# kylittle/Crucible

Hardware: AMD Instinct MI355X
Metric: Msamples/sec (whole node) + achieved HBM GB/s, book1 1920×1080 @ 1/2/4/8 GPU (higher is better)
Workload: dtype f64

## Files before the change

crucible_amd/csrc/pathtrace.hpp:

```cpp
#pragma once
#include <hip/hip_runtime.h>
#include <stddef.h>
#include <stdint.h>
#include <type_traits>

#define CR_HD __host__ __device__ __forceinline__
#define CR_D __device__ __forceinline__
#include "fastdiv.hpp"
#include "residency.hpp"

namespace cr {

template <typename real> struct RealTraits;
template <> struct RealTraits<float> {
    static constexpr float eps = 1.1920928955078125e-07f;
    static constexpr float tiny = 0.0f;
    static constexpr float pi = 3.14159265358979323846f;
};
template <> struct RealTraits<double> {
    static constexpr double eps = 2.220446049250313e-16;
    static constexpr double tiny = 1e-160;
    static constexpr double pi = 3.14159265358979323846;
};

// ... 283 lines not shown
    f.from = from;
    V3<real> w = unit(sub(from, at));
    V3<real> u = unit(cross(c.vup, w));
    V3<real> v = cross(w, u);
    V3<real> vu = scale(c.viewport_width, u);
    V3<real> vv = scale(c.viewport_height, neg(v));
    f.pdu = divs(vu, (real)c.W);
    f.pdv = divs(vv, (real)c.H);
    V3<real> ul = sub(from, scale(c.focus_dist, w));
    ul = sub(ul, divs(vu, real(2)));
    ul = sub(ul, divs(vv, real(2)));
    f.p00 = add(ul, scale(real(0.5), add(f.pdu, f.pdv)));
    f.ddu = scale(c.defocus_radius, u);
    f.ddv = scale(c.defocus_radius, v);
    return f;
}

#if defined(__HIPCC__)

#ifdef CR_DIAG
enum { DG_BOX_WAVE = 0, DG_BOX_LANE, DG_PRIM_WAVE, DG_PRIM_LANE, DG_ROUND_WAVE, DG_ROUND_LANE, DG_LEAFPH_WAVE, DG_LEAFPH_LANE,
       DG_SHADE_WAVE, DG_SHADE_LANE, DG_LAMB_LANE, DG_METAL_LANE, DG_DIEL_LANE, DG_SKY_LANE, DG_RUV_WAVE, DG_RUV_LANE,
       DG_REGEN_WAVE, DG_REGEN_LANE, DG_OUTER_WAVE, DG_UNWIND_WAVE, DG_UNWIND_LANE, DG_HITSH_WAVE, DG_HITSH_LANE, DG_BAND_WAVE, DG_BAND_LANE,
       DG_ROOT2_WAVE, DG_ROOT2_LANE, DG_QUOT_WAVE, DG_QUOT_LANE, DG_QUOTDIV_WAVE, DG_QUOTDIV_LANE, DG_N };
struct Diag { uint32_t v[DG_N]; };
#define CR_DIAG_LEADER() ((threadIdx.x & 63u) == (uint32_t)(__ffsll((unsigned long long)__ballot(1)) - 1))
#define CR_DIAG_HIT(dg, wave_i, lane_i) do { if (dg) { (dg)->v[lane_i]++; if (CR_DIAG_LEADER()) (dg)->v[wave_i]++; } } while (0)
#define CR_DIAG_LANE(dg, lane_i) do { if (dg) (dg)->v[lane_i]++; } while (0)
#else
struct Diag {};
#define CR_DIAG_HIT(dg, wave_i, lane_i) ((void)0)
#define CR_DIAG_LANE(dg, lane_i) ((void)0)
#endif

template <typename real> struct Hit {
    real t;
    int32_t prim;
};

template <typename real>
CR_D bool box_hit(const real* b, V3<real> o, V3<real> inv, real tmin, real tmax) {
    real t0 = (b[0] - o.x) * inv.x, t1 = (b[1] - o.x) * inv.x;
    real nmin, nmax;
    if (t0 < t1) { nmin = t0 > tmin ? t0 : tmin; nmax = t1 < tmax ? t1 : tmax; }
    else { nmin = t1 > tmin ? t1 : tmin; nmax = t0 < tmax ? t0 : tmax; }
    tmin = nmin; tmax = nmax;
    t0 = (b[2] - o.y) * inv.y; t1 = (b[3] - o.y) * inv.y;
// ... 226 lines not shown
template <typename real> CR_HD real soft_acos(real x) {
    using K = TrigK<real>;
    const real ax = r_abs(x);
    if (ax < real(0.5)) { const real z = x * x; return K::pio2_hi - (x - (K::pio2_lo - x * (z * K::S(z)))); }
    if (!(ax <= real(1))) return (x - x) / (x - x);
    if (x < real(0)) {
        const real t = (real(1) + x) * real(0.5);
        const real s = r_sqrt(t);
        const real w = (t * K::S(t)) * s - K::pio2_lo;
        return K::pi_hi - real(2) * (s + w);
    }
    const real t = (real(1) - x) * real(0.5);
    const real s = r_sqrt(t);
    return real(2) * (s + s * (t * K::S(t)));
}
CR_D float r_atan2(float y, float x) { return soft_atan2(y, x); }
CR_D float r_asin(float x) { return soft_asin(x); }
CR_D float r_acos(float x) { return soft_acos(x); }
#define CR_D_CALL static __device__ __attribute__((noinline))
CR_D_CALL double r_atan2(double y, double x) { return soft_atan2(y, x); }
CR_D_CALL double r_asin(double x) { return soft_asin(x); }
CR_D_CALL double r_acos(double x) { return soft_acos(x); }

CR_D float screen_coord(uint64_t u) {
    return (float)((int32_t)(uint32_t)(u >> 40) - (int32_t)(1 << 23)) * 0x1.0p-23f;
}
template <typename real> CR_D V3<real> random_unit_vector_dev(uint64_t& s) {
    if constexpr (!std::is_same<real, double>::value) return random_unit_vector<real>(s);
    else {
        uint64_t ux, uy, uz;
        for (;;) {
            ux = rng_next(s); uy = rng_next(s); uz = rng_next(s);
            const float fx = screen_coord(ux), fy = screen_coord(uy), fz = screen_coord(uz);
            const float lf = __builtin_fmaf(fz, fz, __builtin_fmaf(fy, fy, fx * fx));
            if (lf > 1.0f + 1e-5f) continue;
            if (lf > 1e-5f && lf < 1.0f - 1e-5f) break;
            const double x = -1.0 + 2.0 * u01(ux, 0.0), y = -1.0 + 2.0 * u01(uy, 0.0), z = -1.0 + 2.0 * u01(uz, 0.0);
            const double lensq = x * x + y * y + z * z;
            if (RealTraits<double>::tiny < lensq && lensq <= 1.0) break;
        }
        const V3<double> p = mk<double>(-1.0 + 2.0 * u01(ux, 0.0), -1.0 + 2.0 * u01(uy, 0.0), -1.0 + 2.0 * u01(uz, 0.0));
        return divs(p, r_sqrt(len2(p)));
    }
}
template <typename real> CR_D void random_in_unit_disk_dev(uint64_t& s, real& px, real& py) {
    if constexpr (!std::is_same<real, double>::value) {
        for (;;) {
            px = rng_range<real>(s, real(-1), real(1));
            py = rng_range<real>(s, real(-1), real(1));
            if (px * px + py * py + real(0) * real(0) < real(1)) break;
        }
    } else {
        uint64_t ux, uy;
        for (;;) {
            ux = rng_next(s); uy = rng_next(s);
            const float fx = screen_coord(ux), fy = screen_coord(uy);
            const float lf = __builtin_fmaf(fy, fy, fx * fx);
            if (lf > 1.0f + 1e-5f) continue;
            if (lf < 1.0f - 1e-5f) break;
            const double x = -1.0 + 2.0 * u01(ux, 0.0), y = -1.0 + 2.0 * u01(uy, 0.0);
            if (x * x + y * y + 0.0 * 0.0 < 1.0) break;
        }
        px = -1.0 + 2.0 * u01(ux, 0.0); py = -1.0 + 2.0 * u01(uy, 0.0);
    }
}

template <typename real, bool ANIM, bool CAMK = false>
CR_D void camera_ray(const KernelArgs<real>& A, uint32_t pix_i, uint32_t pix_j, int32_t sample, uint64_t& rng, V3<real>& ro, V3<real>& rd,
                     real& rtime, real current_time) {
    const CamConst<real>& cam = A.cam;
    uint32_t pixel = pix_j * (uint32_t)cam.W + pix_i;
    rng = rng_key(A.seed_mixed, pixel, (uint32_t)sample);
    real ts = current_time + rng_range<real>(rng, real(0), A.shutter_length);
    real ox = rng_uniform<real>(rng) - real(0.5);
    real oy = rng_uniform<real>(rng) - real(0.5);
    CamFrame<real> f;
    if ((ANIM || CAMK) && cam.animated) {
        real fx = cam.from.x, fy = cam.from.y, fz = cam.from.z, fw = real(1);
        real ax = cam.at.x, ay = cam.at.y, az = cam.at.z, aw = real(1);
        timeline_eval(A.cam_keys + cam.from_key_first, cam.from_key_count, ts, fx, fy, fz, fw);
        timeline_eval(A.cam_keys + cam.at_key_first, cam.at_key_count, ts, ax, ay, az, aw);
        f = camera_frame(cam, mk<real>(fw * fx, fw * fy, fw * fz), mk<real>(aw * ax, aw * ay, aw * az));
    } else {
        f.from = cam.from; f.p00 = cam.p00; f.pdu = cam.pdu; f.pdv = cam.pdv; f.ddu = cam.ddu; f.ddv = cam.ddv;
    }
    V3<real> ps = add(add(f.p00, scale((real)pix_i + ox, f.pdu)), scale((real)pix_j + oy, f.pdv));
    V3<real> orig = f.from;
    if (cam.defocus_on) {
        real px, py;
        random_in_unit_disk_dev<real>(rng, px, py);
        orig = add(add(f.from, scale(px, f.ddu)), scale(py, f.ddv));
    }
    ro = orig; rd = sub(ps, orig); rtime = ts;
}
template <typename real, bool ANIM, bool CAMK = false>
CR_D void camera_ray(const KernelArgs<real>& A, uint32_t pix_i, uint32_t pix_j, int32_t sample, uint64_t& rng, V3<real>& ro, V3<real>& rd,
                     real& rtime) {
    camera_ray<real, ANIM, CAMK>(A, pix_i, pix_j, sample, rng, ro, rd, rtime, A.current_time);
}

template <typename T> CR_D T load_rec(const T* p, bool in_lds) {
    static_assert(sizeof(T) % 4 == 0, "records are whole words");
    T out;
    uint32_t* o = reinterpret_cast<uint32_t*>(&out);
    if (in_lds) {
        const __attribute__((address_space(3))) uint32_t* s = (const __attribute__((address_space(3))) uint32_t*)(const void*)p;
        for (size_t k = 0; k < sizeof(T) / 4; k++) o[k] = s[k];
    } else {
        const __attribute__((address_space(1))) uint32_t* s = (const __attribute__((address_space(1))) uint32_t*)(const void*)p;
        for (size_t k = 0; k < sizeof(T) / 4; k++) o[k] = s[k];
    }
    return out;
}

#define CR_CHECKER_LEAF(tex_at, ti, tx, p)                                                                                          \
    for (int guard = 0; guard < 32 && tx.kind == 1; guard++) {                                                                   \
        int32_t s = (int32_t)((uint32_t)as_i32(r_floor(tx.inv_scale * p.x)) + (uint32_t)as_i32(r_floor(tx.inv_scale * p.y)) +   \
                              (uint32_t)as_i32(r_floor(tx.inv_scale * p.z)));                                                      \
        ti = (s % 2 == 0) ? tx.even : tx.odd;                                                                                    \
        tx = tex_at(ti);                                                                                                         \
    }

template <typename real, bool ANIM, bool SIDE_SPLIT = false, bool RELAX = false>
CR_D bool shade(const KernelArgs<real>& A, const Prim<real>* prims, const Mat<real>* mats, const Tex<real>* texs, V3<real>& ro, V3<real>& rd,
                real rtime, uint64_t& rng, int32_t& depth_left, int32_t& stack_n, real best_t, int32_t best, uint32_t stack_stride,
                uint32_t stack_slot, uint32_t& c_tex, V3<real>& col, Diag* dg = nullptr, V3<real>* thr = nullptr) {
    CR_DIAG_HIT(dg, DG_SHADE_WAVE, DG_SHADE_LANE);
    if (best >= 0) {
        CR_DIAG_HIT(dg, DG_HITSH_WAVE, DG_HITSH_LANE);
        const Prim<real>& p = prims[best];
        V3<real> loc = add(ro, scale(best_t, rd));
        V3<real> n;
        real tu = 0, tv = 0;
        auto mat_at = [&](int32_t i) { return SIDE_SPLIT ? load_rec(mats + i, A.lds_side != 0) : mats[i]; };
        auto tex_at = [&](int32_t i) { return SIDE_SPLIT ? load_rec(texs + i, A.lds_side != 0) : texs[i]; };
        const Mat<real> m = mat_at(p.mat());
        bool need_uv = false;
        int32_t leaf_tex = -1;
        if (m.kind == 0 && m.tex >= 0) {
            int ti = m.tex;
            Tex<real> tx = tex_at(ti);
            CR_CHECKER_LEAF(tex_at, ti, tx, loc)
            need_uv = tx.kind == 2;
            leaf_tex = ti;
        }
        if (p.kind() == 0) {
            real g0 = p.g[0], g1 = p.g[1], g2 = p.g[2], g3 = p.g[3];
            if (ANIM && p.key_count) {
                timeline_eval(A.keys + p.key_first, p.key_count, rtime, g0, g1, g2, g3);
                n = divs(sub(loc, mk<real>(g0, g1, g2)), g3);
            } else n = scale(p.g[4], sub(loc, mk<real>(g0, g1, g2)));
            if (need_uv) {
                real theta = r_acos(-n.y);
                real phi = r_atan2(-n.z, n.x) + RealTraits<real>::pi;
                tu = phi / (real(2) * RealTraits<real>::pi);
                tv = theta / RealTraits<real>::pi;
            }
        } else {
            V3<real> a = mk<real>(p.g[0], p.g[1], p.g[2]), b = mk<real>(p.g[3], p.g[4], p.g[5]), c = mk<real>(p.g[6], p.g[7], p.g[8]);
            if (ANIM && p.key_count) {
                a = timeline_vertex(A.keys + p.key_first, p.key_count, rtime, a);
                b = timeline_vertex(A.keys + p.key_first, p.key_count, rtime, b);
                c = timeline_vertex(A.keys + p.key_first, p.key_count, rtime, c);
            }
            n = unit(cross(sub(b, a), sub(c, a)));
            tu = 0; tv = 0;
        }
        bool front = dot(rd, n) < real(0);
        if (!front) n = neg(n);

        V3<real> att = mk<real>(0, 0, 0), ndir = rd;
        bool some;
        V3<real> ruv = mk<real>(0, 0, 0);
#ifdef CR_DIAG
        if (m.kind != 2) {
            for (;;) {
                CR_DIAG_HIT(dg, DG_RUV_WAVE, DG_RUV_LANE);
                real x = rng_range<real>(rng, real(-1), real(1)), y = rng_range<real>(rng, real(-1), real(1)), z = rng_range<real>(rng, real(-1), real(1));
                V3<real> pp = mk<real>(x, y, z);
                real lensq = len2(pp);
                if (RealTraits<real>::tiny < lensq && lensq <= real(1)) { ruv = divs(pp, r_sqrt(lensq)); break; }
            }
        }
        CR_DIAG_LANE(dg, m.kind == 0 ? DG_LAMB_LANE : (m.kind == 1 ? DG_METAL_LANE : DG_DIEL_LANE));
#else
        if (m.kind != 2) ruv = random_unit_vector_dev<real>(rng);
#endif
        if (m.kind == 0) {
            V3<real> dir = add(n, ruv);
            real tol = real(1e-8);
            if (r_abs(dir.x) < tol && r_abs(dir.y) < tol && r_abs(dir.z) < tol) dir = n;
            V3<real> tc;
            if (m.tex < 0) tc = mk<real>(m.albedo[0], m.albedo[1], m.albedo[2]);
            else {
                const Tex<real> lt = tex_at(leaf_tex);
                if (need_uv) tc = image_lookup(A.images, A.texels, lt.image, tu, tv, c_tex);
                else tc = mk<real>(lt.color[0], lt.color[1], lt.color[2]);
            }
            att = c_scale(m.aux, (m.param < real(0)) ? c_neg(tc) : tc);
            ndir = dir;
            if (__ballot(!(m.param >= real(1))) == 0ull) { rng_step(rng); some = true; }
            else some = rng_uniform<real>(rng) <= m.param;
        } else if (m.kind == 1) {
            V3<real> refl = reflect(rd, n);
            refl = add(unit(refl), scale(m.param, ruv));
            att = mk<real>(m.albedo[0], m.albedo[1], m.albedo[2]);
            ndir = refl;
            some = dot(refl, n) > real(0);
        } else {
            att = mk<real>(1, 1, 1);
// ... 164 lines not shown
}

template <typename real> struct WalkState {
    V3<real> inv;
    real dd;
    real rda;
    real best_t;
    int32_t best;
    int32_t idx;
    bool exact_box;
    int32_t oct;
    int32_t pending;
};

template <bool SHARED = false, typename real> CR_D void walk_begin(WalkState<real>& w, V3<real> rd) {
    w.inv = mk<real>(real(1) / rd.x, real(1) / rd.y, real(1) / rd.z);
    w.exact_box = (r_abs(w.inv.x) == r_inf(real(0))) || (r_abs(w.inv.y) == r_inf(real(0))) || (r_abs(w.inv.z) == r_inf(real(0)));
    w.dd = len2(rd);
    w.rda = SHARED ? shared_rcp(w.dd) : quot_divide<real>();
    w.idx = 0; w.best_t = r_inf(real(0)); w.best = -1; w.pending = -1;
    w.oct = (rd.x < real(0) ? 1 : 0) | (rd.y < real(0) ? 2 : 0) | (rd.z < real(0) ? 4 : 0);
}

CR_D void screen_extents(float ofx, float ofy, float ofz, float ifx, float ify, float ifz, float& mo, float& pmax, float& pmin) {
    mo = r_max(r_max(__builtin_fabsf(ofx), __builtin_fabsf(ofy)), __builtin_fabsf(ofz));
    pmax = r_max(r_max(__builtin_fabsf(ifx), __builtin_fabsf(ify)), __builtin_fabsf(ifz));
    pmin = r_min(r_min(__builtin_fabsf(ifx), __builtin_fabsf(ify)), __builtin_fabsf(ifz));
}
CR_D bool screen_in_range(bool exact_box, float mo, float pmax, float pmin) {
    return !exact_box && pmin >= 0x1.0p-100f && pmax <= 0x1.0p100f && mo <= 0x1.0p100f;
}
CR_D float screen_q(float of, float inv_f) { return __builtin_fabsf(of * inv_f); }
CR_D float screen_th0(float qx, float qy, float qz, float pmax) {
    return __builtin_fmaf(0x1.0p-20f, r_max(r_max(qx, qy), qz), __builtin_fmaf(pmax * 0x1.0p-100f, 0x1.0p-47f, 1e-35f));
}
CR_D float screen_box_d(const float* b, Pair<float> fox, Pair<float> foy, Pair<float> foz, Pair<float> fix, Pair<float> fiy, Pair<float> fiz,
                        float tminf, float tmaxf, float th0, float& th) {
    const Pair<float> tx = __builtin_elementwise_fma(Pair<float>{b[0], b[1]}, fix, -(fox * fix));
    const Pair<float> ty = __builtin_elementwise_fma(Pair<float>{b[2], b[3]}, fiy, -(foy * fiy));
    const Pair<float> tz = __builtin_elementwise_fma(Pair<float>{b[4], b[5]}, fiz, -(foz * fiz));
    const float nx = r_min(tx.x, tx.y), ny = r_min(ty.x, ty.y), nz = r_min(tz.x, tz.y);
    const float fx = r_max(tx.x, tx.y), fy = r_max(ty.x, ty.y), fz = r_max(tz.x, tz.y);
    const float lo = r_max(r_max(nx, ny), r_max(nz, tminf));
    float hi, m;
    asm("v_min_f32_e32 %0, %2, %3\n\tv_min3_f32 %0, %4, %5, %0\n\tv_max_f32_e64 %1, |%6|, |%0|"
        : "=&v"(hi), "=v"(m) : "v"(fz), "v"(tmaxf), "v"(fx), "v"(fy), "v"(lo));
    th = __builtin_fmaf(0x1.0p-20f, m, th0);
    return hi - lo;
}
CR_D bool screen_box_miss_exact(const float* b, Pair<float> fox, Pair<float> foy, Pair<float> foz, Pair<float> fix, Pair<float> fiy,
                                Pair<float> fiz, float tminf, float tmaxf) {
    const Pair<float> tx = (Pair<float>{b[0], b[1]} - fox) * fix;
    const Pair<float> ty = (Pair<float>{b[2], b[3]} - foy) * fiy;
    const Pair<float> tz = (Pair<float>{b[4], b[5]} - foz) * fiz;
    const float nx = r_min(tx.x, tx.y), ny = r_min(ty.x, ty.y), nz = r_min(tz.x, tz.y);
    const float fx = r_max(tx.x, tx.y), fy = r_max(ty.x, ty.y), fz = r_max(tz.x, tz.y);
    const float lo = r_max(r_max(nx, ny), r_max(nz, tminf));
    float hi;
    asm("v_min_f32_e32 %0, %1, %2\n\tv_min3_f32 %0, %3, %4, %0" : "=&v"(hi) : "v"(fz), "v"(tmaxf), "v"(fx), "v"(fy));
    return hi <= lo;
}

template <typename real, int RES, bool ANIM, bool SCREEN> constexpr int quot_form() {
    constexpr bool fits = std::is_same<real, double>::value && !ANIM && SCREEN && RES != RES_GLOBAL;
#ifdef CR_QUOT_FORM
    return fits ? CR_QUOT_FORM : 0;
#else
    return fits ? 1 : 0;
#endif
}

template <typename real, int RES, bool ANIM, bool ORD = false, bool SCREEN = false, bool SHARE = false>
CR_D void walk_round(const KernelArgs<real>& A, const Entry<real>* lds_entries, const Prim<real>* prims, V3<real> ro, V3<real> rd, real rtime,
                     WalkState<real>& w, bool walking, uint32_t budget, unsigned long long& c_node, uint32_t& c_prim, Diag* dg = nullptr,
                     const void* lds_screen = nullptr) {
    constexpr bool EXACT = std::is_same<real, float>::value;
    static_assert(!(SCREEN && EXACT && ORD), "the f32 kernels use ScreenEntry records for unordered trees only");
    const real tmin = real(0.001);
    const int32_t n_entries = A.n_entries;
    constexpr int RES64 = SCREEN ? RES_GLOBAL : RES;
    const int32_t lds_n64 = SCREEN ? 0 : A.lds_entries;
    int32_t leaf = w.pending;
    if (walking && leaf < 0) {
        CR_DIAG_HIT(dg, DG_ROUND_WAVE, DG_ROUND_LANE);
        uint32_t exact_steps = w.exact_box ? 0xffffffffu : 0u;
        if constexpr (SCREEN) {
            const float ofx = (float)ro.x, ofy = (float)ro.y, ofz = (float)ro.z;
            const float ifx = (float)w.inv.x, ify = (float)w.inv.y, ifz = (float)w.inv.z;
            float mo, pmax, pmin;
            screen_extents(ofx, ofy, ofz, ifx, ify, ifz, mo, pmax, pmin);
            bool screened;
// ... 134 lines not shown
            if constexpr (RES != RES_LDS && !ANIM) {
                constexpr uint32_t touch = sizeof(Prim<real>) == 96 ? 20u : (uint32_t)(sizeof(Prim<real>) / 4 - 1);
                static_assert((touch + 1) * 4 <= sizeof(Prim<real>), "the touched word must lie inside the record");
                GlobPtr<uint32_t> nx = (GlobPtr<uint32_t>)(const void*)(prims + first + (count - 1));
                const uint32_t t0 = nx[0], t1 = nx[touch];
                test(first);
                asm volatile("" :: "v"(t0), "v"(t1));
                if (count == 2) test(first + 1);
            } else
            for (int32_t k = 0; k < count; k++) test(first + k);
        } else {
            const int32_t first = A.leaf_runs[2 * (leaf & kLeafRunIndex)], count = A.leaf_runs[2 * (leaf & kLeafRunIndex) + 1];
            for (int32_t k = 0; k < count; k++) test(first + k);
        }
    }
}

#ifdef CR_DIAG
#define CR_DIAG_ONLY(...) __VA_ARGS__
#else
#define CR_DIAG_ONLY(...)
#endif

enum : int { ST_NEED_PIXEL = 0, ST_NEED_SAMPLE = 1, ST_TRACE = 2, ST_DONE = 3, ST_WALK = 4, ST_SHADE = 5 };

template <typename real> struct MaxBlock { static constexpr int value = 1024; };

CR_D uint32_t wave_rank(uint64_t ballot) {
    return __builtin_amdgcn_mbcnt_hi((uint32_t)(ballot >> 32), __builtin_amdgcn_mbcnt_lo((uint32_t)ballot, 0u));
}

template <typename real> CR_D const KernelArgs<real>& kernel_args() {
    return *(const KernelArgs<real>*)(const __attribute__((address_space(4))) KernelArgs<real>*)__builtin_amdgcn_kernarg_segment_ptr();
}
template <typename real, int RES, bool ANIM, bool ORD, bool CAMK = false, bool RELAX = false, bool SCREEN = false, bool REG = true, bool LIST = false>
CR_D void pathtrace_body(const KernelArgs<real>& A) {
    using EntryT = typename EntryOf<real, ORD>::type;
    constexpr bool BATCH = RELAX && (ANIM || CAMK);
    constexpr bool REGION = BATCH && REG;
    const KernelArgs<real>& RG = kernel_args<real>();
    extern __shared__ __attribute__((aligned(16))) unsigned char smem[];
#ifdef CR_HOLD_VCC
    unsigned long long vcc_hold;
    asm volatile("s_mov_b64 %0, 0" : "={vcc}"(vcc_hold));
#endif
    const Entry<real>* lds_entries = nullptr;
    const void* lds_screen = nullptr;
// ... 79 lines not shown
            }
            __builtin_amdgcn_fence(__ATOMIC_SEQ_CST, "wavefront");
        }
    };
    const uint32_t total_work = (A.sg_on || RELAX) ? A.sg_total : A.tiles_x * A.tiles_y * 64u;
    const CamConst<real>& cam = A.cam;
    uint32_t wv_next = 0, wv_end = 0;
    const uint32_t SG_CHUNK = A.sg_chunk;

    int state = ST_NEED_PIXEL;
    uint32_t pix_i = 0, pix_j = 0;
    uint32_t item = 0;
    int32_t sample = 0;
    real acc_r = 0, acc_g = 0, acc_b = 0;
    V3<real> ro = mk<real>(0, 0, 0), rd = mk<real>(0, 0, 1);
    real rtime = 0;
    uint64_t rng = 0;
    int32_t depth_left = 0, stack_n = 0;
    uint32_t c_seg = 0, c_prim = 0, c_tex = 0;
    unsigned long long c_node = 0;
    WalkState<real> ws;
    ws.inv = mk<real>(0, 0, 0); ws.dd = 0; ws.rda = quot_divide<real>(); ws.best_t = 0; ws.best = -1; ws.idx = 0; ws.exact_box = false; ws.pending = -1;
    const int32_t n_entries = A.n_entries;

    Diag* dgp = nullptr;
    CR_DIAG_ONLY(Diag dg_store; for (int i = 0; i < DG_N; i++) dg_store.v[i] = 0; dgp = &dg_store;
                 unsigned long long d_t_regen = 0, d_t_trace = 0, d_t_shade = 0;
                 unsigned long long d_t0 = __builtin_readcyclecounter(); const unsigned long long d_begin = d_t0;)
    for (;;) {
        CR_DIAG_ONLY(if (CR_DIAG_LEADER()) dg_store.v[DG_OUTER_WAVE]++; d_t0 = __builtin_readcyclecounter();)
        uint64_t need = __ballot(state == ST_NEED_PIXEL);
        if (need && (A.sg_on || RELAX)) {
            const uint32_t cnt = (uint32_t)__popcll(need), avail = wv_end - wv_next;
            uint32_t fresh = 0;
            uint32_t my_tile = kFxNoTile;
            if (cnt > avail) {
                const int leader = __ffsll((unsigned long long)need) - 1;
                if ((int)lane == leader) fresh = atomicAdd(A.work_counter, SG_CHUNK);
                fresh = (uint32_t)__builtin_amdgcn_readlane((int)fresh, leader);
            }
            if (state == ST_NEED_PIXEL) {
                const uint32_t rank = wave_rank(need);
                const uint32_t w = rank < avail ? wv_next + rank : fresh + (rank - avail);
                if (w >= total_work) state = ST_DONE;
                else {
                    item = w;
// ... 35 lines not shown
            uint32_t cnt = (uint32_t)__popcll(need);
            uint32_t base = 0;
            int leader = __ffsll((unsigned long long)need) - 1;
            if ((int)lane == leader) base = atomicAdd(A.work_counter, cnt);
            base = (uint32_t)__builtin_amdgcn_readlane((int)base, leader);
            if (state == ST_NEED_PIXEL) {
                uint32_t rank = wave_rank(need);
                uint32_t w = base + rank;
                if (w >= total_work) state = ST_DONE;
                else {
                    uint32_t tile = w >> 6, in = w & 63u;
                    uint32_t tx, ty;
                    tile_xy(A, tile, tx, ty);
                    pix_i = tx * 8u + (in & 7u);
                    pix_j = ty * 8u + (in >> 3);
                    if (pix_i < (uint32_t)cam.W && pix_j < (uint32_t)cam.H) {
                        state = ST_NEED_SAMPLE; sample = A.sample_begin; acc_r = acc_g = acc_b = 0;
                    }
                }
            }
        }
        if (__ballot(state != ST_DONE) == 0) break;

        if (state == ST_NEED_SAMPLE) {
            CR_DIAG_HIT(dgp, DG_REGEN_WAVE, DG_REGEN_LANE);
            if constexpr (BATCH) {
                const uint32_t f = batch_frame(A, REGION ? pix_j - RG.reg_y0 : pix_j);
                camera_ray<real, ANIM, CAMK>(A, pix_i, pix_j - f * (A.tiles_y << A.sg_lh), sample, rng, ro, rd, rtime,
                                             A.n_frames > 1u ? A.frame_times[f] : A.current_time);
            } else camera_ray<real, ANIM, CAMK>(A, pix_i, pix_j, sample, rng, ro, rd, rtime);
            depth_left = A.max_depth; stack_n = 0;
            if constexpr (RELAX) thr = mk<real>(1, 1, 1);
            state = ST_TRACE;
        }

        CR_DIAG_ONLY({ unsigned long long t = __builtin_readcyclecounter(); d_t_regen += t - d_t0; d_t0 = t; })
        V3<real> col = mk<real>(0, 0, 0);
        bool finished = false;
        if (state == ST_TRACE) {
            if (depth_left == 0) finished = true;
            else {
                c_seg++;
                walk_begin<quot_form<real, RES, ANIM, SCREEN>() == 1>(ws, rd);
                state = n_entries > 0 ? ST_WALK : ST_SHADE;
            }
        }
        if (__ballot(state == ST_WALK)) {
            for (;;) {
                walk_round<real, RES, ANIM, ORD, SCREEN, true>(A, lds_entries, prims, ro, rd, rtime, ws, state == ST_WALK, A.walk_round_steps, c_node, c_prim, dgp, lds_screen);
                if (state == ST_WALK && ws.idx >= n_entries && ws.pending < 0) state = ST_SHADE;
                const uint64_t walking = __ballot(state == ST_WALK);
                if (!walking || 64u - (uint32_t)__popcll(walking) >= A.walk_exit_lanes) break;
            }
        }
        const bool tracing = (state == ST_SHADE);

        CR_DIAG_ONLY({ unsigned long long t = __builtin_readcyclecounter(); d_t_trace += t - d_t0; d_t0 = t; })
        if (tracing) {
            finished = shade<real, ANIM, RES == RES_TOP, RELAX>(A, prims, mats, texs, ro, rd, rtime, rng, depth_left, stack_n, ws.best_t, ws.best,
                                         A.n_threads, gtid, c_tex, col, dgp, &thr);
            state = ST_TRACE;
        }

        if (RELAX && finished) {
            if constexpr (RELAX) {
                const bool black = col.x == real(0) && col.y == real(0) && col.z == real(0);
                if (!black) {
                    uint32_t ri = pix_i, rj = pix_j;
                    if constexpr (REGION) { ri -= RG.reg_x0; rj -= RG.reg_y0; }
                    const uint32_t tile = (rj >> A.sg_lh) * A.tiles_x + (ri >> A.sg_lw);
                    const uint32_t px = ((rj & ((1u << A.sg_lh) - 1u)) << A.sg_lw) | (ri & ((1u << A.sg_lw) - 1u));
                    const real cc[3] = {col.x, col.y, col.z};
                    unsigned long long v[3];
#pragma unroll
                    for (int c = 0; c < 3; c++) {
                        const double x = (double)cc[c];
                        v[c] = (x == x) ? (unsigned long long)(__builtin_bit_cast(long long, __builtin_fma(x, A.fx_scale, 0x1.0p52)) - 0x4330000000000000ll) : kFxNaN;
                    }
                    const bool nan = (v[0] | v[1] | v[2]) >> 63;
                    unsigned long long* dst;
                    bool in_lds = true;
                    if (tile == fx_tile0) dst = fx_slots + px * 3u;
                    else if (tile == fx_tile1) dst = fx_slots + fx_words + px * 3u;
                    else {
// ... 144 lines not shown
```

crucible_amd/csrc/render.hpp:

```cpp
#pragma once
#include "handle.hpp"

#include <type_traits>

namespace cr {

template <typename real>
int32_t fx_finalize(CrHandle* h, const unsigned long long* sums, real* out, size_t n, double inv_scale, double count, int32_t output_sum) {
    hipLaunchKernelGGL((fx_finalize_kernel<real>), dim3((unsigned)((n + 255) / 256)), dim3(256), 0, h->stream, sums, out, n, inv_scale, count, output_sum);
    HIP_TRY(h, hipGetLastError());
    return CR_OK;
}

#ifdef CR_DIAG
inline int32_t diag_dump(CrHandle* h, int block, uint32_t grid) {
    uint64_t d[64];
    HIP_TRY(h, hipMemcpy(d, h->counters.p, sizeof d, hipMemcpyDeviceToHost));
    const char* names[] = {"box_wave", "box_lane", "prim_wave", "prim_lane", "round_wave", "round_lane", "leafph_wave", "leafph_lane",
                           "shade_wave", "shade_lane", "lamb_lane", "metal_lane", "diel_lane", "sky_lane", "ruv_wave", "ruv_lane",
                           "regen_wave", "regen_lane", "outer_wave", "unwind_wave", "unwind_lane", "hitsh_wave", "hitsh_lane", "band_wave", "band_lane",
                           "root2_wave", "root2_lane", "quot_wave", "quot_lane", "quotdiv_wave", "quotdiv_lane"};
    static_assert(sizeof names / sizeof names[0] == DG_N, "one name per DG_ counter");
    fprintf(stderr, "[diag] block=%d grid=%u clk_regen=%llu clk_trace=%llu clk_shade=%llu clk_total=%llu", block, grid,
            (unsigned long long)d[9], (unsigned long long)d[10], (unsigned long long)d[11], (unsigned long long)d[12]);
    for (int i = 0; i < DG_N; i++) fprintf(stderr, " %s=%llu", names[i], (unsigned long long)d[16 + i]);
    fprintf(stderr, "\n");
    return CR_OK;
}
#endif

template <typename real, int RES, bool ANIM, bool ORD = false, bool LATENCY = false, bool CAMK = false, bool RELAX = false, bool SCREEN = false, bool LIST = false>
int32_t launch(CrHandle* h, const KernelArgs<real>& args_in, size_t scene_lds_bytes, CrStats* stats, const FrameBatch<real>& fb) {
    constexpr bool LDS = RES != RES_GLOBAL || RELAX;
    static_assert(!LATENCY || RES == RES_TOP, "the 6-waves-per-SIMD entry point exists for RES_TOP only");
    KernelArgs<real> args = args_in;
    void (*kern)(const KernelArgs<real>) = pathtrace_kernel<real, RES, ANIM, ORD, CAMK, RELAX, SCREEN>;
    if constexpr (LATENCY) kern = pathtrace_kernel_latency<real, ANIM, ORD, CAMK, RELAX>;
    if constexpr (LIST) kern = pathtrace_kernel_listed<real, RES, ANIM, ORD, CAMK, SCREEN>;
    static_assert(!LIST || (RELAX && ANIM != CAMK && !LATENCY), "the listed kernels are relaxed kernels with keys");
    const int max_block = LATENCY ? LatencyBlock : MaxBlock<real>::value;
    const int32_t n_samples = fb.ad ? fb.ad->pass_samples : args.sample_end - args.sample_begin;
    int tile_lw = h->sg_lw, tile_lh = h->sg_lh;
    if (fb.ad && (tile_lw > fb.ad->block_log2 || tile_lh > fb.ad->block_log2)) tile_lw = tile_lh = -1;
    if (tile_lw < 0) default_tile(n_samples, tile_lw, tile_lh);
    const size_t fx_off = RES != RES_GLOBAL ? ((scene_lds_bytes + 15) & ~(size_t)15) : 0;
// ... 176 lines not shown
```

Before: 4807.

## Merge lens-disk and scatter-sphere rejection samplers into one divergence-shared loop

Splits camera ray generation and hit shading into begin/finish phases so that lanes needing a lens-disk draw (fresh samples) and lanes needing a unit-sphere draw (hit scatter) run the same rejection-sampling loop together instead of in two separately divergent loops. Hit data is parked in the walk-state registers between the trace and the new scatter state. This is meant to cut wavefront divergence from the two rejection loops in the f64 screen-space path. In exchange it adds an extra state-machine step per bounce, more register pressure from the packed hit record, and a material reload.

```diff
diff --git a/crucible_amd/csrc/pathtrace.hpp b/crucible_amd/csrc/pathtrace.hpp
--- a/crucible_amd/csrc/pathtrace.hpp
+++ b/crucible_amd/csrc/pathtrace.hpp
@@ -329,7 +329,8 @@
 enum { DG_BOX_WAVE = 0, DG_BOX_LANE, DG_PRIM_WAVE, DG_PRIM_LANE, DG_ROUND_WAVE, DG_ROUND_LANE, DG_LEAFPH_WAVE, DG_LEAFPH_LANE,
        DG_SHADE_WAVE, DG_SHADE_LANE, DG_LAMB_LANE, DG_METAL_LANE, DG_DIEL_LANE, DG_SKY_LANE, DG_RUV_WAVE, DG_RUV_LANE,
        DG_REGEN_WAVE, DG_REGEN_LANE, DG_OUTER_WAVE, DG_UNWIND_WAVE, DG_UNWIND_LANE, DG_HITSH_WAVE, DG_HITSH_LANE, DG_BAND_WAVE, DG_BAND_LANE,
-       DG_ROOT2_WAVE, DG_ROOT2_LANE, DG_QUOT_WAVE, DG_QUOT_LANE, DG_QUOTDIV_WAVE, DG_QUOTDIV_LANE, DG_N };
+       DG_ROOT2_WAVE, DG_ROOT2_LANE, DG_QUOT_WAVE, DG_QUOT_LANE, DG_QUOTDIV_WAVE, DG_QUOTDIV_LANE, DG_LENS_WAVE, DG_LENS_LANE, DG_LATE_WAVE, DG_LATE_LANE,
+       DG_N };
 struct Diag { uint32_t v[DG_N]; };
 #define CR_DIAG_LEADER() ((threadIdx.x & 63u) == (uint32_t)(__ffsll((unsigned long long)__ballot(1)) - 1))
 #define CR_DIAG_HIT(dg, wave_i, lane_i) do { if (dg) { (dg)->v[lane_i]++; if (CR_DIAG_LEADER()) (dg)->v[wave_i]++; } } while (0)
@@ -602,9 +603,41 @@
 CR_D_CALL double r_asin(double x) { return soft_asin(x); }
 CR_D_CALL double r_acos(double x) { return soft_acos(x); }
 
-CR_D float screen_coord(uint64_t u) {
+#endif
+CR_HD float screen_coord(uint64_t u) {
     return (float)((int32_t)(uint32_t)(u >> 40) - (int32_t)(1 << 23)) * 0x1.0p-23f;
 }
+CR_HD V3<double> unit_vector_of_draws(uint64_t ux, uint64_t uy, uint64_t uz) {
+    const V3<double> p = mk<double>(-1.0 + 2.0 * u01(ux, 0.0), -1.0 + 2.0 * u01(uy, 0.0), -1.0 + 2.0 * u01(uz, 0.0));
+    return divs(p, r_sqrt(len2(p)));
+}
+CR_HD void disk_of_draws(uint64_t ux, uint64_t uy, double& px, double& py) { px = -1.0 + 2.0 * u01(ux, 0.0); py = -1.0 + 2.0 * u01(uy, 0.0); }
+
+enum : int { ROLE_NONE = 0, ROLE_DISK = 1, ROLE_SPHERE = 2 };
+CR_HD bool role_round(uint64_t& s, bool sphere, uint64_t& ux, uint64_t& uy, uint64_t& uz) {
+    ux = rng_next(s); uy = rng_next(s);
+    const float fx = screen_coord(ux), fy = screen_coord(uy);
+    float lf = __builtin_fmaf(fy, fy, fx * fx);
+    if (sphere) {
+        uz = rng_next(s);
+        const float fz = screen_coord(uz);
+        lf = __builtin_fmaf(fz, fz, lf);
+    }
+    if (lf > 1.0f + 1e-5f) return false;
+    if (lf < 1.0f - 1e-5f && (!sphere || lf > 1e-5f)) return true;
+    const double x = -1.0 + 2.0 * u01(ux, 0.0), y = -1.0 + 2.0 * u01(uy, 0.0);
+    if (sphere) {
+        const double z = -1.0 + 2.0 * u01(uz, 0.0);
+        const double lensq = x * x + y * y + z * z;
+        return RealTraits<double>::tiny < lensq && lensq <= 1.0;
+    }
+    return x * x + y * y + 0.0 * 0.0 < 1.0;
+}
+CR_HD void random_role_draws(uint64_t& s, int role, uint64_t& ux, uint64_t& uy, uint64_t& uz) {
+    bool open = role != ROLE_NONE;
+    while (open) open = !role_round(s, role == ROLE_SPHERE, ux, uy, uz);
+}
+#if defined(__HIPCC__)
 template <typename real> CR_D V3<real> random_unit_vector_dev(uint64_t& s) {
     if constexpr (!std::is_same<real, double>::value) return random_unit_vector<real>(s);
     else {
@@ -619,8 +652,7 @@
             const double lensq = x * x + y * y + z * z;
             if (RealTraits<double>::tiny < lensq && lensq <= 1.0) break;
         }
-        const V3<double> p = mk<double>(-1.0 + 2.0 * u01(ux, 0.0), -1.0 + 2.0 * u01(uy, 0.0), -1.0 + 2.0 * u01(uz, 0.0));
-        return divs(p, r_sqrt(len2(p)));
+        return unit_vector_of_draws(ux, uy, uz);
     }
 }
 template <typename real> CR_D void random_in_unit_disk_dev(uint64_t& s, real& px, real& py) {
@@ -641,19 +673,34 @@
             const double x = -1.0 + 2.0 * u01(ux, 0.0), y = -1.0 + 2.0 * u01(uy, 0.0);
             if (x * x + y * y + 0.0 * 0.0 < 1.0) break;
         }
-        px = -1.0 + 2.0 * u01(ux, 0.0); py = -1.0 + 2.0 * u01(uy, 0.0);
-    }
-}
-
-template <typename real, bool ANIM, bool CAMK = false>
+        disk_of_draws(ux, uy, px, py);
+    }
+}
+#ifdef CR_DIAG
+template <typename real> CR_D void random_in_unit_disk_counted(uint64_t& s, real& px, real& py, Diag* dg) {
+    for (;;) {
+        CR_DIAG_HIT(dg, DG_LENS_WAVE, DG_LENS_LANE);
+        px = rng_range<real>(s, real(-1), real(1));
+        py = rng_range<real>(s, real(-1), real(1));
+        if (px * px + py * py + real(0) * real(0) < real(1)) break;
+    }
+}
+#endif
+
+enum : int { CAM_WHOLE = 0, CAM_BEGIN = 1, CAM_FINISH = 2 };
+template <typename real, bool ANIM, bool CAMK = false, int PART = CAM_WHOLE>
 CR_D void camera_ray(const KernelArgs<real>& A, uint32_t pix_i, uint32_t pix_j, int32_t sample, uint64_t& rng, V3<real>& ro, V3<real>& rd,
-                     real& rtime, real current_time) {
+                     real& rtime, real current_time, Diag* dg = nullptr, real lens_x = real(0), real lens_y = real(0)) {
     const CamConst<real>& cam = A.cam;
-    uint32_t pixel = pix_j * (uint32_t)cam.W + pix_i;
-    rng = rng_key(A.seed_mixed, pixel, (uint32_t)sample);
-    real ts = current_time + rng_range<real>(rng, real(0), A.shutter_length);
-    real ox = rng_uniform<real>(rng) - real(0.5);
-    real oy = rng_uniform<real>(rng) - real(0.5);
+    real ts, ox, oy;
+    if constexpr (PART != CAM_FINISH) {
+        uint32_t pixel = pix_j * (uint32_t)cam.W + pix_i;
+        rng = rng_key(A.seed_mixed, pixel, (uint32_t)sample);
+        ts = current_time + rng_range<real>(rng, real(0), A.shutter_length);
+        ox = rng_uniform<real>(rng) - real(0.5);
+        oy = rng_uniform<real>(rng) - real(0.5);
+        if constexpr (PART == CAM_BEGIN) { rtime = ts; rd.x = ox; rd.y = oy; return; }
+    } else { ts = rtime; ox = rd.x; oy = rd.y; }
     CamFrame<real> f;
     if ((ANIM || CAMK) && cam.animated) {
         real fx = cam.from.x, fy = cam.from.y, fz = cam.from.z, fw = real(1);
@@ -667,16 +714,22 @@
     V3<real> ps = add(add(f.p00, scale((real)pix_i + ox, f.pdu)), scale((real)pix_j + oy, f.pdv));
     V3<real> orig = f.from;
     if (cam.defocus_on) {
-        real px, py;
-        random_in_unit_disk_dev<real>(rng, px, py);
+        real px = lens_x, py = lens_y;
+        if constexpr (PART == CAM_WHOLE) {
+#ifdef CR_DIAG
+            random_in_unit_disk_counted<real>(rng, px, py, dg);
+#else
+            random_in_unit_disk_dev<real>(rng, px, py);
+#endif
+        }
         orig = add(add(f.from, scale(px, f.ddu)), scale(py, f.ddv));
     }
     ro = orig; rd = sub(ps, orig); rtime = ts;
 }
 template <typename real, bool ANIM, bool CAMK = false>
 CR_D void camera_ray(const KernelArgs<real>& A, uint32_t pix_i, uint32_t pix_j, int32_t sample, uint64_t& rng, V3<real>& ro, V3<real>& rd,
-                     real& rtime) {
-    camera_ray<real, ANIM, CAMK>(A, pix_i, pix_j, sample, rng, ro, rd, rtime, A.current_time);
+                     real& rtime, Diag* dg = nullptr) {
+    camera_ray<real, ANIM, CAMK>(A, pix_i, pix_j, sample, rng, ro, rd, rtime, A.current_time, dg);
 }
 
 template <typename T> CR_D T load_rec(const T* p, bool in_lds) {
@@ -701,71 +754,93 @@
         tx = tex_at(ti);                                                                                                         \
     }
 
-template <typename real, bool ANIM, bool SIDE_SPLIT = false, bool RELAX = false>
+enum : int { SHADE_WHOLE = 0, SHADE_BEGIN = 1, SHADE_SCATTER = 2 };
+template <typename real> struct ShadeHit {
+    V3<real> loc;
+    V3<real> n;
+    real tu, tv;
+    Mat<real> m;
+    int32_t mat;
+    int32_t leaf_tex;
+    bool need_uv, front;
+};
+template <typename real, bool ANIM, bool SIDE_SPLIT = false, bool RELAX = false, int PART = SHADE_WHOLE>
 CR_D bool shade(const KernelArgs<real>& A, const Prim<real>* prims, const Mat<real>* mats, const Tex<real>* texs, V3<real>& ro, V3<real>& rd,
                 real rtime, uint64_t& rng, int32_t& depth_left, int32_t& stack_n, real best_t, int32_t best, uint32_t stack_stride,
-                uint32_t stack_slot, uint32_t& c_tex, V3<real>& col, Diag* dg = nullptr, V3<real>* thr = nullptr) {
-    CR_DIAG_HIT(dg, DG_SHADE_WAVE, DG_SHADE_LANE);
-    if (best >= 0) {
-        CR_DIAG_HIT(dg, DG_HITSH_WAVE, DG_HITSH_LANE);
-        const Prim<real>& p = prims[best];
-        V3<real> loc = add(ro, scale(best_t, rd));
-        V3<real> n;
+                uint32_t stack_slot, uint32_t& c_tex, V3<real>& col, Diag* dg = nullptr, V3<real>* thr = nullptr, ShadeHit<real>* hit = nullptr,
+                V3<real> ruv_drawn = V3<real>{0, 0, 0}) {
+    if constexpr (PART != SHADE_SCATTER) CR_DIAG_HIT(dg, DG_SHADE_WAVE, DG_SHADE_LANE);
+    if (PART == SHADE_SCATTER || best >= 0) {
+        if constexpr (PART != SHADE_SCATTER) CR_DIAG_HIT(dg, DG_HITSH_WAVE, DG_HITSH_LANE);
+        const Prim<real>& p = prims[PART == SHADE_SCATTER ? 0 : best];
+        V3<real> loc, n;
         real tu = 0, tv = 0;
+        bool need_uv = false, front;
+        int32_t leaf_tex = -1;
         auto mat_at = [&](int32_t i) { return SIDE_SPLIT ? load_rec(mats + i, A.lds_side != 0) : mats[i]; };
         auto tex_at = [&](int32_t i) { return SIDE_SPLIT ? load_rec(texs + i, A.lds_side != 0) : texs[i]; };
-        const Mat<real> m = mat_at(p.mat());
-        bool need_uv = false;
-        int32_t leaf_tex = -1;
-        if (m.kind == 0 && m.tex >= 0) {
-            int ti = m.tex;
-            Tex<real> tx = tex_at(ti);
-            CR_CHECKER_LEAF(tex_at, ti, tx, loc)
-            need_uv = tx.kind == 2;
-            leaf_tex = ti;
-        }
-        if (p.kind() == 0) {
-            real g0 = p.g[0], g1 = p.g[1], g2 = p.g[2], g3 = p.g[3];
-            if (ANIM && p.key_count) {
-                timeline_eval(A.keys + p.key_first, p.key_count, rtime, g0, g1, g2, g3);
-                n = divs(sub(loc, mk<real>(g0, g1, g2)), g3);
-            } else n = scale(p.g[4], sub(loc, mk<real>(g0, g1, g2)));
-            if (need_uv) {
-                real theta = r_acos(-n.y);
-                real phi = r_atan2(-n.z, n.x) + RealTraits<real>::pi;
-                tu = phi / (real(2) * RealTraits<real>::pi);
-                tv = theta / RealTraits<real>::pi;
-            }
+        const Mat<real> m = [&]() { if constexpr (PART == SHADE_SCATTER) return hit->m; else return mat_at(p.mat()); }();
+        if constexpr (PART == SHADE_SCATTER) {
+            loc = hit->loc; n = hit->n; tu = hit->tu; tv = hit->tv; need_uv = hit->need_uv; front = hit->front; leaf_tex = hit->leaf_tex;
         } else {
-            V3<real> a = mk<real>(p.g[0], p.g[1], p.g[2]), b = mk<real>(p.g[3], p.g[4], p.g[5]), c = mk<real>(p.g[6], p.g[7], p.g[8]);
-            if (ANIM && p.key_count) {
-                a = timeline_vertex(A.keys + p.key_first, p.key_count, rtime, a);
-                b = timeline_vertex(A.keys + p.key_first, p.key_count, rtime, b);
-                c = timeline_vertex(A.keys + p.key_first, p.key_count, rtime, c);
-            }
-            n = unit(cross(sub(b, a), sub(c, a)));
-            tu = 0; tv = 0;
-        }
-        bool front = dot(rd, n) < real(0);
-        if (!front) n = neg(n);
+            loc = add(ro, scale(best_t, rd));
+            if (m.kind == 0 && m.tex >= 0) {
+                int ti = m.tex;
+                Tex<real> tx = tex_at(ti);
+                CR_CHECKER_LEAF(tex_at, ti, tx, loc)
+                need_uv = tx.kind == 2;
+                leaf_tex = ti;
+            }
+            if (p.kind() == 0) {
+                real g0 = p.g[0], g1 = p.g[1], g2 = p.g[2], g3 = p.g[3];
+                if (ANIM && p.key_count) {
+                    timeline_eval(A.keys + p.key_first, p.key_count, rtime, g0, g1, g2, g3);
+                    n = divs(sub(loc, mk<real>(g0, g1, g2)), g3);
+                } else n = scale(p.g[4], sub(loc, mk<real>(g0, g1, g2)));
+                if (need_uv) {
+                    real theta = r_acos(-n.y);
+                    real phi = r_atan2(-n.z, n.x) + RealTraits<real>::pi;
+                    tu = phi / (real(2) * RealTraits<real>::pi);
+                    tv = theta / RealTraits<real>::pi;
+                }
+            } else {
+                V3<real> a = mk<real>(p.g[0], p.g[1], p.g[2]), b = mk<real>(p.g[3], p.g[4], p.g[5]), c = mk<real>(p.g[6], p.g[7], p.g[8]);
+                if (ANIM && p.key_count) {
+                    a = timeline_vertex(A.keys + p.key_first, p.key_count, rtime, a);
+                    b = timeline_vertex(A.keys + p.key_first, p.key_count, rtime, b);
+                    c = timeline_vertex(A.keys + p.key_first, p.key_count, rtime, c);
+                }
+                n = unit(cross(sub(b, a), sub(c, a)));
+                tu = 0; tv = 0;
+            }
+            front = dot(rd, n) < real(0);
+            if (!front) n = neg(n);
+            if constexpr (PART == SHADE_BEGIN) {
+                hit->loc = loc; hit->n = n; hit->tu = tu; hit->tv = tv; hit->m = m; hit->mat = p.mat(); hit->need_uv = need_uv; hit->front = front;
+                hit->leaf_tex = leaf_tex;
+                return false;
+            }
+        }
 
         V3<real> att = mk<real>(0, 0, 0), ndir = rd;
         bool some;
-        V3<real> ruv = mk<real>(0, 0, 0);
+        V3<real> ruv = PART == SHADE_SCATTER ? ruv_drawn : mk<real>(0, 0, 0);
+        if constexpr (PART != SHADE_SCATTER) {
 #ifdef CR_DIAG
-        if (m.kind != 2) {
-            for (;;) {
-                CR_DIAG_HIT(dg, DG_RUV_WAVE, DG_RUV_LANE);
-                real x = rng_range<real>(rng, real(-1), real(1)), y = rng_range<real>(rng, real(-1), real(1)), z = rng_range<real>(rng, real(-1), real(1));
-                V3<real> pp = mk<real>(x, y, z);
-                real lensq = len2(pp);
-                if (RealTraits<real>::tiny < lensq && lensq <= real(1)) { ruv = divs(pp, r_sqrt(lensq)); break; }
-            }
+            if (m.kind != 2) {
+                for (;;) {
+                    CR_DIAG_HIT(dg, DG_RUV_WAVE, DG_RUV_LANE);
+                    real x = rng_range<real>(rng, real(-1), real(1)), y = rng_range<real>(rng, real(-1), real(1)), z = rng_range<real>(rng, real(-1), real(1));
+                    V3<real> pp = mk<real>(x, y, z);
+                    real lensq = len2(pp);
+                    if (RealTraits<real>::tiny < lensq && lensq <= real(1)) { ruv = divs(pp, r_sqrt(lensq)); break; }
+                }
+            }
+#else
+            if (m.kind != 2) ruv = random_unit_vector_dev<real>(rng);
+#endif
         }
         CR_DIAG_LANE(dg, m.kind == 0 ? DG_LAMB_LANE : (m.kind == 1 ? DG_METAL_LANE : DG_DIEL_LANE));
-#else
-        if (m.kind != 2) ruv = random_unit_vector_dev<real>(rng);
-#endif
         if (m.kind == 0) {
             V3<real> dir = add(n, ruv);
             real tol = real(1e-8);
@@ -976,6 +1051,20 @@
     w.oct = (rd.x < real(0) ? 1 : 0) | (rd.y < real(0) ? 2 : 0) | (rd.z < real(0) ? 4 : 0);
 }
 
+CR_D void hit_park(WalkState<double>& w, const ShadeHit<double>& h) {
+    w.inv = h.n; w.dd = h.tu; w.rda = h.tv; w.best = h.mat;
+    const uint32_t bits = (uint32_t)h.m.kind | (h.front ? 4u : 0u) | (h.need_uv ? 8u : 0u);
+    w.best_t = __builtin_bit_cast(double, ((uint64_t)(uint32_t)h.leaf_tex << 32) | (uint64_t)bits);
+}
+CR_D ShadeHit<double> hit_parked(const WalkState<double>& w) {
+    ShadeHit<double> h;
+    const uint64_t b = __builtin_bit_cast(uint64_t, w.best_t);
+    h.n = w.inv; h.tu = w.dd; h.tv = w.rda; h.mat = w.best;
+    h.m.kind = (int32_t)((uint32_t)b & 3u); h.front = ((uint32_t)b & 4u) != 0u; h.need_uv = ((uint32_t)b & 8u) != 0u;
+    h.leaf_tex = (int32_t)(uint32_t)(b >> 32);
+    return h;
+}
+
 CR_D void screen_extents(float ofx, float ofy, float ofz, float ifx, float ify, float ifz, float& mo, float& pmax, float& pmin) {
     mo = r_max(r_max(__builtin_fabsf(ofx), __builtin_fabsf(ofy)), __builtin_fabsf(ofz));
     pmax = r_max(r_max(__builtin_fabsf(ifx), __builtin_fabsf(ify)), __builtin_fabsf(ifz));
@@ -1021,6 +1110,15 @@
     return fits ? CR_QUOT_FORM : 0;
 #else
     return fits ? 1 : 0;
+#endif
+}
+
+template <typename real, int RES, bool ANIM, bool SCREEN> constexpr bool merged_samplers() {
+    constexpr bool fits = std::is_same<real, double>::value && !ANIM && SCREEN && RES != RES_GLOBAL;
+#ifdef CR_MERGED_SAMPLERS
+    return fits && CR_MERGED_SAMPLERS != 0;
+#else
+    return fits;
 #endif
 }
 
@@ -1201,7 +1299,7 @@
 #define CR_DIAG_ONLY(...)
 #endif
 
-enum : int { ST_NEED_PIXEL = 0, ST_NEED_SAMPLE = 1, ST_TRACE = 2, ST_DONE = 3, ST_WALK = 4, ST_SHADE = 5 };
+enum : int { ST_NEED_PIXEL = 0, ST_NEED_SAMPLE = 1, ST_TRACE = 2, ST_DONE = 3, ST_WALK = 4, ST_SHADE = 5, ST_SCATTER = 6 };
 
 template <typename real> struct MaxBlock { static constexpr int value = 1024; };
 
@@ -1327,6 +1425,7 @@
     WalkState<real> ws;
     ws.inv = mk<real>(0, 0, 0); ws.dd = 0; ws.rda = quot_divide<real>(); ws.best_t = 0; ws.best = -1; ws.idx = 0; ws.exact_box = false; ws.pending = -1;
     const int32_t n_entries = A.n_entries;
+    constexpr bool MERGED = merged_samplers<real, RES, ANIM, SCREEN>();
 
     Diag* dgp = nullptr;
     CR_DIAG_ONLY(Diag dg_store; for (int i = 0; i < DG_N; i++) dg_store.v[i] = 0; dgp = &dg_store;
@@ -1408,23 +1507,65 @@
         }
         if (__ballot(state != ST_DONE) == 0) break;
 
-        if (state == ST_NEED_SAMPLE) {
+        V3<real> col = mk<real>(0, 0, 0);
+        bool finished = false;
+        if constexpr (MERGED) {
+            const bool fresh = state == ST_NEED_SAMPLE, hit = state == ST_SCATTER;
+            uint32_t cam_j = pix_j;
+            if constexpr (BATCH) { if (fresh) cam_j -= batch_frame(A, REGION ? pix_j - RG.reg_y0 : pix_j) * (A.tiles_y << A.sg_lh); }
+            if (fresh) {
+                CR_DIAG_HIT(dgp, DG_REGEN_WAVE, DG_REGEN_LANE);
+                if constexpr (BATCH) {
+                    const uint32_t f = batch_frame(A, REGION ? pix_j - RG.reg_y0 : pix_j);
+                    camera_ray<real, ANIM, CAMK, CAM_BEGIN>(A, pix_i, cam_j, sample, rng, ro, rd, rtime, A.n_frames > 1u ? A.frame_times[f] : A.current_time);
+                } else camera_ray<real, ANIM, CAMK, CAM_BEGIN>(A, pix_i, pix_j, sample, rng, ro, rd, rtime, A.current_time);
+            }
+            ShadeHit<real> sh = hit_parked(ws);
+            const int role = (fresh && cam.defocus_on) ? ROLE_DISK : ((hit && sh.m.kind != 2) ? ROLE_SPHERE : ROLE_NONE);
+            uint64_t ux = 0, uy = 0, uz = 0;
+#ifdef CR_DIAG
+            for (bool open = role != ROLE_NONE; open;) {
+                CR_DIAG_HIT(dgp, DG_RUV_WAVE, DG_RUV_LANE);
+                if (role == ROLE_DISK) CR_DIAG_HIT(dgp, DG_LENS_WAVE, DG_LENS_LANE);
+                open = !role_round(rng, role == ROLE_SPHERE, ux, uy, uz);
+            }
+#else
+            random_role_draws(rng, role, ux, uy, uz);
+#endif
+            if (hit) {
+                const V3<real> ruv = role == ROLE_SPHERE ? unit_vector_of_draws(ux, uy, uz) : mk<real>(0, 0, 0);
+                sh.loc = ro;
+                sh.m = RES == RES_TOP ? load_rec(mats + sh.mat, A.lds_side != 0) : mats[sh.mat];
+                finished = shade<real, ANIM, RES == RES_TOP, RELAX, SHADE_SCATTER>(A, prims, mats, texs, ro, rd, rtime, rng, depth_left, stack_n, real(0), 0,
+                                                                                  A.n_threads, gtid, c_tex, col, dgp, &thr, &sh, ruv);
+                if (finished) CR_DIAG_HIT(dgp, DG_LATE_WAVE, DG_LATE_LANE);
+                else state = ST_TRACE;
+            } else if (fresh) {
+                real px = 0, py = 0;
+                if (role == ROLE_DISK) disk_of_draws(ux, uy, px, py);
+                camera_ray<real, ANIM, CAMK, CAM_FINISH>(A, pix_i, cam_j, sample, rng, ro, rd, rtime, real(0), dgp, px, py);
+                depth_left = A.max_depth; stack_n = 0;
+                if constexpr (RELAX) thr = mk<real>(1, 1, 1);
+                state = ST_TRACE;
+            }
+        } else if (state == ST_NEED_SAMPLE) {
             CR_DIAG_HIT(dgp, DG_REGEN_WAVE, DG_REGEN_LANE);
             if constexpr (BATCH) {
                 const uint32_t f = batch_frame(A, REGION ? pix_j - RG.reg_y0 : pix_j);
                 camera_ray<real, ANIM, CAMK>(A, pix_i, pix_j - f * (A.tiles_y << A.sg_lh), sample, rng, ro, rd, rtime,
-                                             A.n_frames > 1u ? A.frame_times[f] : A.current_time);
-            } else camera_ray<real, ANIM, CAMK>(A, pix_i, pix_j, sample, rng, ro, rd, rtime);
+                                             A.n_frames > 1u ? A.frame_times[f] : A.current_time, dgp);
+            } else camera_ray<real, ANIM, CAMK>(A, pix_i, pix_j, sample, rng, ro, rd, rtime, dgp);
             depth_left = A.max_depth; stack_n = 0;
             if constexpr (RELAX) thr = mk<real>(1, 1, 1);
             state = ST_TRACE;
         }
 
         CR_DIAG_ONLY({ unsigned long long t = __builtin_readcyclecounter(); d_t_regen += t - d_t0; d_t0 = t; })
-        V3<real> col = mk<real>(0, 0, 0);
-        bool finished = false;
         if (state == ST_TRACE) {
-            if (depth_left == 0) finished = true;
+            if (depth_left == 0) {
+                finished = true;
+                if constexpr (MERGED) CR_DIAG_HIT(dgp, DG_LATE_WAVE, DG_LATE_LANE);
+            }
             else {
                 c_seg++;
                 walk_begin<quot_form<real, RES, ANIM, SCREEN>() == 1>(ws, rd);
@@ -1443,9 +1584,22 @@
 
         CR_DIAG_ONLY({ unsigned long long t = __builtin_readcyclecounter(); d_t_trace += t - d_t0; d_t0 = t; })
         if (tracing) {
-            finished = shade<real, ANIM, RES == RES_TOP, RELAX>(A, prims, mats, texs, ro, rd, rtime, rng, depth_left, stack_n, ws.best_t, ws.best,
-                                         A.n_threads, gtid, c_tex, col, dgp, &thr);
-            state = ST_TRACE;
+            if constexpr (MERGED) {
+                if (ws.best < 0)
+                    finished = shade<real, ANIM, RES == RES_TOP, RELAX, SHADE_BEGIN>(A, prims, mats, texs, ro, rd, rtime, rng, depth_left, stack_n, ws.best_t, -1,
+                                                                                    A.n_threads, gtid, c_tex, col, dgp, &thr);
+                if (ws.best >= 0) {
+                    ShadeHit<real> sh;
+                    shade<real, ANIM, RES == RES_TOP, RELAX, SHADE_BEGIN>(A, prims, mats, texs, ro, rd, rtime, rng, depth_left, stack_n, ws.best_t, ws.best,
+                                                                         A.n_threads, gtid, c_tex, col, dgp, &thr, &sh);
+                    hit_park(ws, sh); ro = sh.loc;
+                }
+                state = ST_SCATTER;
+            } else {
+                finished = shade<real, ANIM, RES == RES_TOP, RELAX>(A, prims, mats, texs, ro, rd, rtime, rng, depth_left, stack_n, ws.best_t, ws.best,
+                                             A.n_threads, gtid, c_tex, col, dgp, &thr);
+                state = ST_TRACE;
+            }
         }
 
         if (RELAX && finished) {
diff --git a/crucible_amd/csrc/render.hpp b/crucible_amd/csrc/render.hpp
--- a/crucible_amd/csrc/render.hpp
+++ b/crucible_amd/csrc/render.hpp
@@ -19,8 +19,9 @@
     const char* names[] = {"box_wave", "box_lane", "prim_wave", "prim_lane", "round_wave", "round_lane", "leafph_wave", "leafph_lane",
                            "shade_wave", "shade_lane", "lamb_lane", "metal_lane", "diel_lane", "sky_lane", "ruv_wave", "ruv_lane",
                            "regen_wave", "regen_lane", "outer_wave", "unwind_wave", "unwind_lane", "hitsh_wave", "hitsh_lane", "band_wave", "band_lane",
-                           "root2_wave", "root2_lane", "quot_wave", "quot_lane", "quotdiv_wave", "quotdiv_lane"};
+                           "root2_wave", "root2_lane", "quot_wave", "quot_lane", "quotdiv_wave", "quotdiv_lane", "lens_wave", "lens_lane", "late_wave", "late_lane"};
     static_assert(sizeof names / sizeof names[0] == DG_N, "one name per DG_ counter");
+    static_assert(16 + DG_N <= sizeof d / sizeof d[0], "the DG_ counters follow word 16 of the handle's 64 counter words");
     fprintf(stderr, "[diag] block=%d grid=%u clk_regen=%llu clk_trace=%llu clk_shade=%llu clk_total=%llu", block, grid,
             (unsigned long long)d[9], (unsigned long long)d[10], (unsigned long long)d[11], (unsigned long long)d[12]);
     for (int i = 0; i < DG_N; i++) fprintf(stderr, " %s=%llu", names[i], (unsigned long long)d[16 + i]);
```

Result: no change. 4851, median of 6 (+0.9%).
